# massquantity/LibRecommender

Hardware: NVIDIA H100
Metric: recommend_user users/sec (all-items top-K) (higher is better)
Workload: dtype f32 scores (fp16 tensor-core candidate pass + exact fp32 re-score)

## Files before the change

### librecommender_b200/csrc/score_topk_tc.cu

```cuda
#include <cmath>
#include <type_traits>
#include "common.cuh"
#include "ptx_sm90.cuh"
#include "../../include/b200reco.h"
#include <cuda_fp16.h>

namespace b200 {
namespace tc {

constexpr int TM = 128;
constexpr int TN = 256;
constexpr int KBLK = 64;
constexpr int CAPG_MAX = 256;
constexpr int GW = 8;
constexpr int REC = 12;
constexpr int NB = 1024;
constexpr int STEP = 64;
constexpr int W_PRE = 2;
constexpr int KROW_MAX = 288;
constexpr int MAX_KB = 4;
constexpr int PRE_STRIDE = 8;
constexpr double PRE_DELTA = 1e-5;
constexpr int PRE_TIE_ALLOWANCE = 16;
constexpr int A_KB_BYTES = TM * KBLK * 2;
constexpr int B_KB_BYTES = TN * KBLK * 2;
constexpr int MAXU = 3072;
constexpr int MAXC = 2048;
constexpr int FIN_THREADS = 256;
constexpr float ERR_COEF = 0.00097705f;

constexpr int SWEEP_CONSUMER_WARPS = 8;
constexpr int WARP_TMA = SWEEP_CONSUMER_WARPS;
constexpr int SWEEP_THREADS = 32 * (SWEEP_CONSUMER_WARPS + 4);
constexpr int SWEEP_PRODUCER_REGS = 40, SWEEP_CONSUMER_REGS = 232;

struct CatalogHeader {
  uint32_t max_norm_bits;
  int32_t d, d_pad;
  int64_t N, N_pad;
  float scale;
  float max_norm_scaled;
};

struct RowMeta {
  float eps2;
  float R;
  float scale;
  int32_t k_row;
  int32_t pre_k;
  int32_t active;
  int32_t apply;
  int32_t capped;
};


struct SweepParams {
  int64_t N;
  int32_t B_pad, m_tiles, n_splits, tiles_per_split, total_tiles, KB, nstage;
  int32_t kb_stages;
  int32_t n_pre_tiles;
  int32_t pre_stride;
  int32_t capg, trig;
  int32_t ablate;
  uint32_t hint_ns;
  const RowMeta* meta;
  uint32_t* row_tau_key;
  int32_t* row_status;
  uint32_t* ghist;
  float* cand_r;
  int32_t* cand_cnt;
  float* blockmax;
};

__device__ __forceinline__ float pow2_scale_for(float nrm) {
  if (!(nrm > 0.f) || !(nrm < 3.0e38f)) return 1.f;
  int x;
  frexpf(nrm, &x);
  int e = 7 - x;
  e = max(-120, min(120, e));
  return ldexpf(1.f, e);
}

__global__ void item_norm_kernel(const float* __restrict__ I, int64_t ldi, int64_t N, int d,
                                 CatalogHeader* hdr) {
  const int64_t row = ((int64_t)blockIdx.x * blockDim.x + threadIdx.x) >> 5;
  const int lane = threadIdx.x & 31;
  if (row >= N) return;
  float ss = 0.f;
  for (int k = lane; k < d; k += 32) {
    const float v = __ldg(I + row * ldi + k);
    ss = fmaf(v, v, ss);
  }
  ss = warp_sum(ss);
  if (lane == 0) atomicMax(&hdr->max_norm_bits, __float_as_uint(sqrtf(ss) * 1.0001f));
}

__global__ void item_scale_kernel(CatalogHeader* hdr) {
  const float mx = __uint_as_float(hdr->max_norm_bits);
  const float s = pow2_scale_for(mx);
  hdr->scale = s;
  hdr->max_norm_scaled = mx * s;
}

__global__ void prep_items_kernel(const float* __restrict__ I, int64_t ldi, int64_t N, int d,
                                  int d_pad, int64_t N_pad, __half* __restrict__ out,
                                  const CatalogHeader* __restrict__ hdr) {
  const int64_t row = ((int64_t)blockIdx.x * blockDim.x + threadIdx.x) >> 5;
  const int lane = threadIdx.x & 31;
  if (row >= N_pad) return;
  const float s = hdr->scale;
  for (int k = lane; k < d_pad; k += 32) {
// ... 534 lines not shown
      if (lane == 0) ptx::mbar_arrive(&ss->a_empty);
    }
  }
  __syncthreads();
  if (CL > 1) ptx::cluster_sync_all();
}

constexpr int GUESS_THREADS = 256;
__global__ void __launch_bounds__(GUESS_THREADS)
guess_kernel(const float* __restrict__ blockmax, int n_vals , int B_pad,
             const RowMeta* __restrict__ meta, uint32_t* __restrict__ row_tau_key,
             uint32_t* __restrict__ guess_key) {
  __shared__ uint32_t hist[32][256 + 1];
  __shared__ uint32_t s_prefix[32], s_krem[32], s_ok[32];
  const int lane = threadIdx.x & 31, wid = threadIdx.x >> 5;
  const int row = blockIdx.x * 32 + lane;
  const RowMeta m = meta[row];
  if (wid == 0) { s_prefix[lane] = 0; s_krem[lane] = (uint32_t)m.pre_k; s_ok[lane] = m.active != 0; }
  for (int pass = 0; pass < 4; ++pass) {
    const int shift = 24 - 8 * pass;
    for (int i = threadIdx.x; i < 32 * 257; i += GUESS_THREADS) (&hist[0][0])[i] = 0;
    __syncthreads();
    const uint32_t prefix = s_prefix[lane];
    for (int i = wid; i < n_vals; i += GUESS_THREADS / 32) {
      const float v = blockmax[(int64_t)i * B_pad + row];
      const uint32_t key = float_to_key(v);
      if (v > -3.0e38f && (pass == 0 || (key >> (shift + 8)) == prefix))
        atomicAdd(&hist[lane][(key >> shift) & 255u], 1u);
    }
    __syncthreads();
    for (int rr = wid; rr < 32; rr += GUESS_THREADS / 32) {
      uint32_t mine[8], tot = 0;
#pragma unroll
      for (int b = 0; b < 8; ++b) { mine[b] = hist[rr][lane * 8 + b]; tot += mine[b]; }
      uint32_t incl = tot;
#pragma unroll
      for (int o = 1; o < 32; o <<= 1) {
        const uint32_t t = __shfl_down_sync(0xffffffffu, incl, o);
        if (lane + o < 32) incl += t;
      }
      const uint32_t excl = incl - tot;
      const uint32_t krem = s_krem[rr];
      const uint32_t total = __shfl_sync(0xffffffffu, incl, 0);
      if (excl < krem && krem <= incl) {
        uint32_t c = excl;
#pragma unroll
        for (int b = 7; b >= 0; --b) {
          if (c + mine[b] >= krem) {
            s_prefix[rr] = (s_prefix[rr] << 8) | (uint32_t)(lane * 8 + b);
            s_krem[rr] = krem - c;
            break;
          }
          c += mine[b];
        }
      }
      if (lane == 0 && total < krem) s_ok[rr] = 0;
    }
    __syncthreads();
  }
  if (wid == 0) {
    const uint32_t key = s_ok[lane] ? s_prefix[lane] : 0u;
    row_tau_key[row] = key;
    guess_key[row] = key;
  }
}

struct FinalizeParams {
  int64_t B, N;
  int32_t B_pad, n_lists, K, d, capg;
  const RowMeta* meta;
  int32_t* row_status;
  const uint32_t* row_tau_key;
  const uint32_t* tau_guess_key;
  const float* cand_r;
  const int32_t* cand_cnt;
  const float* U; int64_t ldu;
  const float* I; int64_t ldi;
  const int64_t* user_ids;
  const int64_t* indptr; const int32_t* idx;
  int64_t* out_ids;
  float* out_scores;
};

__global__ void __launch_bounds__(FIN_THREADS, 5)
finalize_kernel(const FinalizeParams p) {
  __shared__ uint32_t hist[256];
  __shared__ uint32_t s_prefix, s_krem;
  __shared__ uint32_t s_wtot[FIN_THREADS / 32];
  __shared__ int s_nu, s_nc;
  __shared__ float u_s[MAXU];
  __shared__ int32_t u_id[MAXU];
  __shared__ unsigned long long c_sort[MAXC];
  __shared__ float urow[MAX_KB * KBLK];
  int32_t* htab = reinterpret_cast<int32_t*>(c_sort);
  const int tid = threadIdx.x;
  const int64_t row = blockIdx.x;
  int64_t* oid = p.out_ids + row * p.K;
  float* osc = p.out_scores ? p.out_scores + row * p.K : nullptr;
  const RowMeta meta = p.meta[row];
  auto give_up = [&](int code) {
    if (code && tid == 0) p.row_status[row] = code;
    for (int i = tid; i < p.K; i += FIN_THREADS) { oid[i] = -1; if (osc) osc[i] = 0.f; }
  };
  if (p.row_status[row] != 0) { give_up(0); return; }
  const uint32_t tk = p.row_tau_key[row];
  const float low = tk ? key_to_float(tk) : __int_as_float(0xff800000);
  if (tid == 0) { s_nu = 0; s_nc = 0; }
  int* s_cnt = reinterpret_cast<int*>(c_sort);
  int* s_off = s_cnt + p.n_lists;
  for (int s = tid; s < p.n_lists; s += FIN_THREADS) s_cnt[s] = p.cand_cnt[(int64_t)s * p.B_pad + row];
  __syncthreads();
  if (tid < 32) {
    const int per = (p.n_lists + 31) / 32;
    const int b = min(tid * per, p.n_lists), e = min(b + per, p.n_lists);
    int sum = 0;
    for (int s = b; s < e; ++s) sum += s_cnt[s];
    int incl = sum;
#pragma unroll
    for (int o = 1; o < 32; o <<= 1) {
      const int t = __shfl_up_sync(0xffffffffu, incl, o);
      if (tid >= o) incl += t;
    }
    int run = incl - sum;
    for (int s = b; s < e; ++s) { s_off[s] = run; run += s_cnt[s]; }
    if (tid == 31) s_off[p.n_lists] = incl;
  }
  __syncthreads();
  {
    const int lane = tid & 31;
    const int total = s_off[p.n_lists];
    constexpr int UN = 3;
    for (int g0 = 0; g0 < total; g0 += FIN_THREADS * UN) {
      float4 a[UN], b[UN];
      int base[UN];
      bool ok[UN];
#pragma unroll
      for (int q = 0; q < UN; ++q) {
        const int g = g0 + q * FIN_THREADS + tid;
        ok[q] = g < total;
        a[q] = b[q] = make_float4(0.f, 0.f, 0.f, 0.f);
        base[q] = 0;
        if (ok[q]) {
          int lo = 0, hi = p.n_lists - 1;
          while (lo < hi) {
            const int mid = (lo + hi + 1) >> 1;
            if (s_off[mid] <= g) lo = mid; else hi = mid - 1;
          }
          const int j = g - s_off[lo];
          const int64_t slot = (int64_t)lo * p.B_pad + row;
          const float4* ls = reinterpret_cast<const float4*>(p.cand_r + (slot * (int64_t)p.capg + j) * REC);
          a[q] = __ldcs(ls);
          b[q] = __ldcs(ls + 1);
          base[q] = __ldcs(reinterpret_cast<const int32_t*>(ls + 2));
        }
      }
#pragma unroll
      for (int q = 0; q < UN; ++q) {
        const float v[8] = {a[q].x, a[q].y, a[q].z, a[q].w, b[q].x, b[q].y, b[q].z, b[q].w};
#pragma unroll
        for (int e = 0; e < 8; ++e) {
          const bool hit = ok[q] && v[e] >= low && (int64_t)(base[q] + e) < p.N;
          const unsigned m = __ballot_sync(0xffffffffu, hit);
          if (m) {
            int pos0 = 0;
            if (lane == 0) pos0 = atomicAdd(&s_nu, __popc(m));
            pos0 = __shfl_sync(0xffffffffu, pos0, 0);
            const int pos = pos0 + __popc(m & ((1u << lane) - 1u));
            if (hit && pos < MAXU) { u_s[pos] = v[e]; u_id[pos] = base[q] + e; }
          }
        }
      }
    }
  }
  __syncthreads();
  const int nu = s_nu;
  if (nu < meta.k_row) { give_up(2); return; }
  const bool in_smem = nu <= MAXU;
  auto for_each = [&](auto&& f) {
    if (in_smem) {
      for (int i = tid; i < nu; i += FIN_THREADS) f(u_s[i], u_id[i]);
    } else {
      for (int s = 0; s < p.n_lists; ++s) {
        const int64_t slot = (int64_t)s * p.B_pad + row;
        const int n = p.cand_cnt[slot];
        const float* ls = p.cand_r + slot * (int64_t)(p.capg * REC);
        for (int i = tid; i < n * GW; i += FIN_THREADS) {
          const float v = ls[(i / GW) * REC + (i % GW)];
          const int32_t id = reinterpret_cast<const int32_t*>(ls)[(i / GW) * REC + 8] + (i % GW);
          if (v >= low && (int64_t)id < p.N) f(v, id);
        }
      }
    }
  };
  uint32_t prefix = 0, krem = (uint32_t)meta.k_row;
  for (int pass = 0; pass < 4; ++pass) {
    const int shift = 24 - 8 * pass;
    hist[tid] = 0;
    __syncthreads();
    for_each([&](float v, int32_t) {
      const uint32_t key = float_to_key(v);
      if (pass == 0 || (key >> (shift + 8)) == prefix) atomicAdd(&hist[(key >> shift) & 255u], 1u);
    });
    __syncthreads();
    {
      const int lane = tid & 31, wid = tid >> 5;
      const uint32_t v = hist[tid];
      uint32_t incl = v;
#pragma unroll
      for (int o = 1; o < 32; o <<= 1) {
        const uint32_t t = __shfl_down_sync(0xffffffffu, incl, o);
        if (lane + o < 32) incl += t;
      }
      if (lane == 0) s_wtot[wid] = incl;
      __syncthreads();
      uint32_t above = 0;
      for (int w2 = wid + 1; w2 < FIN_THREADS / 32; ++w2) above += s_wtot[w2];
      incl += above;
      const uint32_t excl = incl - v;
      if (excl < krem && krem <= incl) {
        s_prefix = (prefix << 8) | (uint32_t)tid;
        s_krem = krem - excl;
      }
    }
    __syncthreads();
    prefix = s_prefix;
    krem = s_krem;
    __syncthreads();
  }
  const float thr = key_to_float(prefix) - meta.eps2;
  {
    const uint32_t gk = p.tau_guess_key[row];
    if (gk != 0u && key_to_float(gk) > thr) { give_up(3); return; }
  }
  if (in_smem) {
    int my_keep[MAXU / FIN_THREADS];
#pragma unroll
    for (int t = 0; t < MAXU / FIN_THREADS; ++t) {
      const int i = tid + t * FIN_THREADS;
      my_keep[t] = (i < nu && u_s[i] >= thr) ? u_id[i] : -1;
    }
    __syncthreads();
#pragma unroll
    for (int t = 0; t < MAXU / FIN_THREADS; ++t) {
      if (my_keep[t] >= 0) {
        const int pos = atomicAdd(&s_nc, 1);
        if (pos < MAXC) u_id[pos] = my_keep[t];
      }
    }
  } else {
    __syncthreads();
    for_each([&](float v, int32_t id) {
      if (v >= thr) {
        const int pos = atomicAdd(&s_nc, 1);
        if (pos < MAXC) u_id[pos] = id;
      }
    });
  }
  for (int i = tid; i < 2 * MAXC; i += FIN_THREADS) htab[i] = -1;
  __syncthreads();
  const int nc = s_nc;
  int32_t* c_id = u_id;
  if (nc > MAXC || nc < p.K) { give_up(4); return; }
  const int64_t u = p.user_ids[row];
  if (meta.apply) {
    for (int i = tid; i < nc; i += FIN_THREADS) {
      uint32_t h = ((uint32_t)c_id[i] * 2654435761u) & (2 * MAXC - 1);
      while (atomicCAS(&htab[h], -1, i) != -1) h = (h + 1) & (2 * MAXC - 1);
    }
    __syncthreads();
    const int64_t beg = p.indptr[u], end = p.indptr[u + 1];
    for (int64_t j = beg + tid; j < end; j += FIN_THREADS) {
      const int32_t it = p.idx[j];
      uint32_t h = ((uint32_t)it * 2654435761u) & (2 * MAXC - 1);
      while (true) {
        const int32_t e = htab[h];
        if (e < 0) break;
        if (c_id[e] == it || c_id[e] == ~it) { c_id[e] = ~it; break; }
        h = (h + 1) & (2 * MAXC - 1);
      }
    }
  }
  for (int k = tid; k < p.d; k += FIN_THREADS) urow[k] = __ldg(p.U + u * p.ldu + k);
  __syncthreads();
  const bool vec4 = (p.d % 4 == 0) && (p.ldi % 4 == 0) && ((reinterpret_cast<uintptr_t>(p.I) & 15) == 0);
  int P = 1;
  while (P < nc) P <<= 1;
  unsigned long long mine[MAXC / FIN_THREADS];
#pragma unroll
  for (int t = 0; t < MAXC / FIN_THREADS; ++t) {
    const int i = tid + t * FIN_THREADS;
    unsigned long long comp = 0ull;
    if (i < nc && c_id[i] >= 0) {
      const float* it = p.I + (int64_t)c_id[i] * p.ldi;
      float acc = 0.f;
      if (vec4) {
        const float4* it4 = reinterpret_cast<const float4*>(it);
#pragma unroll 8
        for (int k4 = 0; k4 < p.d / 4; ++k4) {
          const float4 x = __ldg(it4 + k4);
          acc = fmaf(urow[4 * k4 + 0], x.x, acc);
          acc = fmaf(urow[4 * k4 + 1], x.y, acc);
          acc = fmaf(urow[4 * k4 + 2], x.z, acc);
          acc = fmaf(urow[4 * k4 + 3], x.w, acc);
        }
      } else {
        for (int k = 0; k < p.d; ++k) acc = fmaf(urow[k], __ldg(it + k), acc);
      }
      comp = ((unsigned long long)float_to_key(acc) << 32) | (unsigned long long)(~(uint32_t)c_id[i]);
    }
    mine[t] = comp;
  }
  __syncthreads();
  if (P <= 2 * FIN_THREADS) {
    auto bitonic_regs = [&](auto ec) {
      constexpr int EPT = decltype(ec)::value;
      unsigned long long x[EPT];
#pragma unroll
      for (int t = 0; t < EPT; ++t) x[t] = mine[t];
      int buf = 0;
#pragma unroll 1
      for (int k = 2; k <= P; k <<= 1) {
#pragma unroll 1
        for (int j = k >> 1; j > 0; j >>= 1) {
          if (EPT == 2 && j >= FIN_THREADS) {
            const unsigned long long a = x[0], b = x[EPT - 1];
            x[0] = a > b ? a : b;
            x[EPT - 1] = a > b ? b : a;
            continue;
          }
          unsigned long long y[EPT];
          if (j >= 32) {
            unsigned long long* sb = c_sort + buf * (EPT * FIN_THREADS);
#pragma unroll
            for (int t = 0; t < EPT; ++t) sb[t * FIN_THREADS + tid] = x[t];
            __syncthreads();
#pragma unroll
            for (int t = 0; t < EPT; ++t) y[t] = sb[t * FIN_THREADS + (tid ^ j)];
            buf ^= 1;
          } else {
#pragma unroll
            for (int t = 0; t < EPT; ++t) y[t] = __shfl_xor_sync(0xffffffffu, x[t], j);
          }
#pragma unroll
          for (int t = 0; t < EPT; ++t) {
            const int e = tid + t * FIN_THREADS;
            const bool take_max = (((e & k) == 0) == ((e & j) == 0));
            x[t] = take_max ? (x[t] > y[t] ? x[t] : y[t]) : (x[t] < y[t] ? x[t] : y[t]);
          }
        }
      }
      __syncthreads();
#pragma unroll
      for (int t = 0; t < EPT; ++t) c_sort[t * FIN_THREADS + tid] = x[t];
      __syncthreads();
    };
    if (P <= FIN_THREADS) bitonic_regs(std::integral_constant<int, 1>{});
    else bitonic_regs(std::integral_constant<int, 2>{});
  } else {
#pragma unroll
    for (int t = 0; t < MAXC / FIN_THREADS; ++t) {
      const int i = tid + t * FIN_THREADS;
      if (i < P) c_sort[i] = mine[t];
    }
    __syncthreads();
    for (int k = 2; k <= P; k <<= 1) {
      for (int j = k >> 1; j > 0; j >>= 1) {
        for (int i = tid; i < P; i += FIN_THREADS) {
          const int ixj = i ^ j;
          if (ixj > i) {
            const unsigned long long a = c_sort[i], b = c_sort[ixj];
            const bool desc = ((i & k) == 0);
            if (desc ? (a < b) : (a > b)) { c_sort[i] = b; c_sort[ixj] = a; }
          }
        }
        __syncthreads();
      }
    }
  }
  {
    const unsigned long long kth = c_sort[p.K - 1];
    const bool short_row = kth == 0ull;
    const bool unsafe = meta.capped && key_to_float((uint32_t)(kth >> 32)) * meta.scale < thr + 0.5f * meta.eps2;
    if (short_row || unsafe) { __syncthreads(); give_up(5); return; }
  }
  for (int i = tid; i < p.K; i += FIN_THREADS) {
    const unsigned long long c = c_sort[i];
    oid[i] = (int64_t)(~(uint32_t)(c & 0xffffffffull));
    if (osc) osc[i] = key_to_float((uint32_t)(c >> 32));
  }
}

typedef CUresult (*EncodeTiledFn)(CUtensorMap*, CUtensorMapDataType, cuuint32_t, void*,
                                  const cuuint64_t*, const cuuint64_t*, const cuuint32_t*,
                                  const cuuint32_t*, CUtensorMapInterleave, CUtensorMapSwizzle,
                                  CUtensorMapL2promotion, CUtensorMapFloatOOBfill);

static EncodeTiledFn get_encode_fn() {
  static EncodeTiledFn fn = nullptr;
  if (fn) return fn;
  void* p = nullptr;
  cudaDriverEntryPointQueryResult q;
  if (cudaGetDriverEntryPoint("cuTensorMapEncodeTiled", &p, cudaEnableDefault, &q) != cudaSuccess ||
      q != cudaDriverEntryPointSuccess)
    return nullptr;
  fn = (EncodeTiledFn)p;
  return fn;
}

static int make_tmap(CUtensorMap* m, const void* base, int64_t rows, int d_pad, int box_rows) {
  EncodeTiledFn enc = get_encode_fn();
  B200_REQUIRE(enc, "cuTensorMapEncodeTiled entry point not available");
  cuuint64_t dims[2] = {(cuuint64_t)d_pad, (cuuint64_t)rows};
  cuuint64_t strides[1] = {(cuuint64_t)d_pad * 2};
  cuuint32_t box[2] = {(cuuint32_t)KBLK, (cuuint32_t)box_rows};
  cuuint32_t estr[2] = {1, 1};
  CUresult r = enc(m, CU_TENSOR_MAP_DATA_TYPE_FLOAT16, 2, const_cast<void*>(base), dims, strides,
                   box, estr, CU_TENSOR_MAP_INTERLEAVE_NONE, CU_TENSOR_MAP_SWIZZLE_128B,
                   CU_TENSOR_MAP_L2_PROMOTION_L2_256B, CU_TENSOR_MAP_FLOAT_OOB_FILL_NONE);
  B200_REQUIRE(r == CUDA_SUCCESS, "cuTensorMapEncodeTiled failed (%d)", (int)r);
  return 0;
}

static inline int pad_to(int64_t x, int m) { return (int)((x + m - 1) / m * m); }
static inline size_t al256(size_t x) { return (x + 255) & ~(size_t)255; }


static int g_epi = 5;
static int g_cluster = 2;
static int g_nh = 1;
static int g_ablate = 0;
static int g_hint_ns = 20000;
static int g_pre_stride = PRE_STRIDE;
static double g_pre_delta = PRE_DELTA;
static float g_pre_coef = 0.f;
static int g_pre_margin = 12;

struct Plan {
  int B_pad, d_pad, KB, m_tiles, total_tiles, n_splits, tiles_per_split, nstage, n_pre_tiles, kb_stages;
  int W, n_lists, capg, trig;
  int CL, NH;
  bool use_pre;
  int pre_stride;
  int pre_sampled;
  int64_t N_pad;
  size_t smem_bytes;
  size_t off_A, off_meta, off_tau, off_guess, off_status, off_cnt, off_hist, off_cs, off_bm, total;
};

static int make_plan(int64_t B, int64_t N, int d, Plan* pl) {
  pl->d_pad = pad_to(d, KBLK);
  pl->KB = pl->d_pad / KBLK;
  B200_REQUIRE(pl->KB >= 1 && pl->KB <= MAX_KB, "fused scorer supports embed width <= %d (got %d)",
               MAX_KB * KBLK, d);
  pl->CL = (g_cluster == 2 && B > TM) ? 2 : 1;
  pl->kb_stages = pl->KB > 2;
  pl->NH = (g_nh == 3 && pl->kb_stages) ? 1 : g_nh;
  pl->B_pad = pad_to(B, TM * pl->CL);
  pl->N_pad = (N + TN - 1) / TN * TN;
  pl->m_tiles = pl->B_pad / TM;
  pl->total_tiles = (int)(pl->N_pad / TN);
  pl->W = 2;
  const int ovh = 12;
  long best = -1;
  int bestS = 1;
  const int sms = num_sms() > 0 ? num_sms() : 132;
  const int maxS = pl->total_tiles < 2 * sms ? pl->total_tiles : 2 * sms;
  for (int S = 1; S <= maxS; ++S) {
    const long units = (long)pl->m_tiles * S;
    const long waves = (units + sms - 1) / sms;
    const long tps = (pl->total_tiles + S - 1) / S;
    const long cost = waves * (tps + ovh);
// ... 199 lines not shown
  out[4] = pl.n_pre_tiles; out[5] = pl.nstage; out[6] = pl.CL * 10 + pl.NH; out[7] = pl.capg;
  if (n_out >= 10) { out[8] = pl.pre_stride; out[9] = pl.pre_sampled; }
  if (n_out >= 10 + KROW_MAX + 1) rank_table(pl, out + 10);
  return 0;
}

extern "C" int b200_recommend_embed_workspace_bytes(int64_t B, int64_t N, int32_t d, int32_t K,
                                                    size_t* bytes) {
  B200_REQUIRE(bytes && B >= 1 && N >= 1 && d >= 1 && K >= 1, "bad arguments");
  Plan pl;
  if (int rc = make_plan(B, N, d, &pl)) return rc;
  *bytes = pl.total;
  return 0;
}

extern "C" int b200_recommend_embed(const float* U, int64_t ldu, const int64_t* user_ids, int64_t B,
                                    const float* I, int64_t ldi, int64_t N, int32_t d,
                                    const void* catalog, const int64_t* indptr, const int32_t* idx,
                                    int64_t n_users, int32_t filter, int32_t K, int64_t* out_ids,
                                    float* out_scores, int32_t* row_status, void* workspace,
                                    size_t workspace_bytes, void* stream_, void* ev_sweep_start,
                                    void* ev_sweep_stop) {
  B200_REQUIRE(U && user_ids && I && catalog && out_ids && row_status && workspace,
               "b200_recommend_embed: null pointer");
  B200_REQUIRE((int64_t)K <= N, "`n_rec` %d exceeds num of items %lld", K, (long long)N);
  B200_REQUIRE(K <= KROW_MAX, "b200_recommend_embed: n_rec %d above the fused-path limit %d", K, KROW_MAX);
  B200_REQUIRE(N < (1ll << 31) - TN, "N too large");
  if (B == 0) return 0;
  cudaStream_t stream = (cudaStream_t)stream_;
  Plan pl;
  if (int rc = make_plan(B, N, d, &pl)) return rc;
  B200_REQUIRE(workspace_bytes >= pl.total, "workspace too small (%zu < %zu)", workspace_bytes, pl.total);
  char* ws = (char*)(((uintptr_t)workspace + 255) & ~(uintptr_t)255);
  __half* A = (__half*)(ws + pl.off_A);
  RowMeta* meta = (RowMeta*)(ws + pl.off_meta);
  uint32_t* tau = (uint32_t*)(ws + pl.off_tau);
  uint32_t* guess = (uint32_t*)(ws + pl.off_guess);
  int32_t* status = (int32_t*)(ws + pl.off_status);
  int32_t* cnt = (int32_t*)(ws + pl.off_cnt);
  uint32_t* ghist = (uint32_t*)(ws + pl.off_hist);
  float* cand_r = (float*)(ws + pl.off_cs);
  float* bm = (float*)(ws + pl.off_bm);
  const CatalogHeader* hdr = (const CatalogHeader*)catalog;
  const __half* Ih = (const __half*)((const char*)catalog + 256);

  PreRank pre_rank;
  rank_table(pl, pre_rank.k);
  prep_users_kernel<<<(unsigned)ceil_div64((int64_t)pl.B_pad * 32, 256), 256, 0, stream>>>(
      U, ldu, user_ids, B, pl.B_pad, d, pl.d_pad, K, N, filter, pre_rank, indptr, n_users, hdr, A, meta,
      tau, status);
  count_launch();
  B200_CUDA_OK(cudaMemsetAsync(cnt, 0, (pl.off_cs - pl.off_cnt), stream));

  CUtensorMap tmA, tmB, tmBh;
  if (int rc = make_tmap(&tmA, A, pl.B_pad, pl.d_pad, TM)) return rc;
  if (int rc = make_tmap(&tmB, Ih, pl.N_pad, pl.d_pad, TN)) return rc;
  if (int rc = make_tmap(&tmBh, Ih, pl.N_pad, pl.d_pad, TN / 2)) return rc;

  SweepParams sp;
  sp.N = N; sp.B_pad = pl.B_pad; sp.m_tiles = pl.m_tiles; sp.n_splits = pl.n_splits;
  sp.tiles_per_split = pl.tiles_per_split; sp.total_tiles = pl.total_tiles; sp.KB = pl.KB;
  sp.nstage = pl.nstage; sp.kb_stages = pl.kb_stages; sp.n_pre_tiles = pl.n_pre_tiles;
  sp.pre_stride = pl.pre_stride; sp.capg = pl.capg; sp.trig = pl.trig;
  sp.meta = meta; sp.row_tau_key = tau;
  sp.row_status = status; sp.ghist = ghist; sp.cand_r = cand_r; sp.cand_cnt = cnt;
  sp.blockmax = bm; sp.ablate = g_ablate; sp.hint_ns = (uint32_t)g_hint_ns;
  const int n_units = pl.m_tiles * pl.n_splits;
  const int sm_count = num_sms();
  int grid = n_units < sm_count ? n_units : sm_count;
  grid -= grid % pl.CL;

  if (ev_sweep_start) B200_CUDA_OK(cudaEventRecord((cudaEvent_t)ev_sweep_start, stream));
  if (pl.use_pre) {
    if (int rc = launch_pre_dispatch(grid, pl, stream, tmA, tmB, tmBh, sp)) return rc;
    guess_kernel<<<(unsigned)(pl.B_pad / 32), GUESS_THREADS, 0, stream>>>(
        bm, W_PRE * pl.n_splits * pl.n_pre_tiles, pl.B_pad, meta, tau, guess);
    count_launch();
  } else {
    B200_CUDA_OK(cudaMemsetAsync(guess, 0, (size_t)pl.B_pad * 4, stream));
  }
  if (int rc = launch_main_dispatch(grid, pl, g_epi, stream, tmA, tmB, tmBh, sp)) return rc;
  if (ev_sweep_stop) B200_CUDA_OK(cudaEventRecord((cudaEvent_t)ev_sweep_stop, stream));

  FinalizeParams fp;
  fp.B = B; fp.N = N; fp.B_pad = pl.B_pad; fp.n_lists = pl.n_lists; fp.K = K; fp.d = d; fp.capg = pl.capg;
  fp.meta = meta; fp.row_status = status; fp.row_tau_key = tau; fp.tau_guess_key = guess;
  fp.cand_r = cand_r; fp.cand_cnt = cnt;
  fp.U = U; fp.ldu = ldu; fp.I = I; fp.ldi = ldi; fp.user_ids = user_ids; fp.indptr = indptr;
  fp.idx = idx; fp.out_ids = out_ids; fp.out_scores = out_scores;
  finalize_kernel<<<(unsigned)B, FIN_THREADS, 0, stream>>>(fp);
  count_launch();
  B200_CUDA_OK(cudaMemcpyAsync(row_status, status, (size_t)B * 4, cudaMemcpyDeviceToDevice, stream));
  B200_CUDA_OK(cudaGetLastError());
  return 0;
}
```

Before: 2.343 million.

## Shrink finalize CTA, use min/max-bounded wide radix select, prefetch user row

The finalize kernel now runs 128-thread CTAs with 7 per SM and a smaller shared union buffer. The radix select starts from the common prefix of the observed min/max keys and uses 12-bit histograms stored in the sort buffer, so it needs fewer passes. The user embedding row and the first interaction id are loaded early to hide their latency, and the register bitonic sort is extended to 4 elements per thread. Rows with more than 1024 candidates now take the slower global-memory path, and the larger histograms add extra clearing and scanning work per pass.

```diff
diff --git a/librecommender_b200/csrc/score_topk_tc.cu b/librecommender_b200/csrc/score_topk_tc.cu
--- a/librecommender_b200/csrc/score_topk_tc.cu
+++ b/librecommender_b200/csrc/score_topk_tc.cu
@@ -24,9 +24,9 @@
 constexpr int PRE_TIE_ALLOWANCE = 16;
 constexpr int A_KB_BYTES = TM * KBLK * 2;
 constexpr int B_KB_BYTES = TN * KBLK * 2;
-constexpr int MAXU = 3072;
+constexpr int MAXU = 1024;
 constexpr int MAXC = 2048;
-constexpr int FIN_THREADS = 256;
+constexpr int FIN_THREADS = 128, FIN_CTAS_PER_SM = 7;
 constexpr float ERR_COEF = 0.00097705f;
 
 constexpr int SWEEP_CONSUMER_WARPS = 8;
@@ -727,30 +727,48 @@
   float* out_scores;
 };
 
-__global__ void __launch_bounds__(FIN_THREADS, 5)
+constexpr int SEL_BITS = 12;
+constexpr int SEL_BINS = 1 << SEL_BITS;
+static_assert(SEL_BINS * 4 <= MAXC * 8, "the select histogram lives in the sort buffer");
+static_assert(2 * MAXU >= MAXC, "the candidate ids live in the union buffer");
+static_assert(SEL_BINS % FIN_THREADS == 0, "whole bins per thread");
+constexpr int FIN_UR = (MAX_KB * KBLK + FIN_THREADS - 1) / FIN_THREADS;
+constexpr int FIN_SORT_REGS = 512;
+
+__global__ void __launch_bounds__(FIN_THREADS, FIN_CTAS_PER_SM)
 finalize_kernel(const FinalizeParams p) {
-  __shared__ uint32_t hist[256];
-  __shared__ uint32_t s_prefix, s_krem;
+  __shared__ uint32_t s_prefix, s_krem, s_kmin, s_kmax;
   __shared__ uint32_t s_wtot[FIN_THREADS / 32];
   __shared__ int s_nu, s_nc;
-  __shared__ float u_s[MAXU];
-  __shared__ int32_t u_id[MAXU];
-  __shared__ unsigned long long c_sort[MAXC];
+  __shared__ int32_t u_buf[2 * MAXU];
+  float* u_s = reinterpret_cast<float*>(u_buf);
+  int32_t* u_id = u_buf + MAXU;
+  __shared__ __align__(16) unsigned long long c_sort[MAXC];
   __shared__ float urow[MAX_KB * KBLK];
   int32_t* htab = reinterpret_cast<int32_t*>(c_sort);
+  uint32_t* hist = reinterpret_cast<uint32_t*>(c_sort);
   const int tid = threadIdx.x;
   const int64_t row = blockIdx.x;
   int64_t* oid = p.out_ids + row * p.K;
   float* osc = p.out_scores ? p.out_scores + row * p.K : nullptr;
+  const int64_t u = p.user_ids[row];
   const RowMeta meta = p.meta[row];
   auto give_up = [&](int code) {
     if (code && tid == 0) p.row_status[row] = code;
     for (int i = tid; i < p.K; i += FIN_THREADS) { oid[i] = -1; if (osc) osc[i] = 0.f; }
   };
   if (p.row_status[row] != 0) { give_up(0); return; }
+  float ur[FIN_UR];
+#pragma unroll
+  for (int t = 0; t < FIN_UR; ++t) {
+    const int k = tid + t * FIN_THREADS;
+    ur[t] = k < p.d ? __ldg(p.U + u * p.ldu + k) : 0.f;
+  }
+  int64_t cbeg = 0, cend = 0;
+  if (meta.apply) { cbeg = p.indptr[u]; cend = p.indptr[u + 1]; }
   const uint32_t tk = p.row_tau_key[row];
   const float low = tk ? key_to_float(tk) : __int_as_float(0xff800000);
-  if (tid == 0) { s_nu = 0; s_nc = 0; }
+  if (tid == 0) { s_nu = 0; s_nc = 0; s_kmin = 0xffffffffu; s_kmax = 0u; }
   int* s_cnt = reinterpret_cast<int*>(c_sort);
   int* s_off = s_cnt + p.n_lists;
   for (int s = tid; s < p.n_lists; s += FIN_THREADS) s_cnt[s] = p.cand_cnt[(int64_t)s * p.B_pad + row];
@@ -771,6 +789,7 @@
     if (tid == 31) s_off[p.n_lists] = incl;
   }
   __syncthreads();
+  uint32_t kmin = 0xffffffffu, kmax = 0u;
   {
     const int lane = tid & 31;
     const int total = s_off[p.n_lists];
@@ -805,6 +824,11 @@
 #pragma unroll
         for (int e = 0; e < 8; ++e) {
           const bool hit = ok[q] && v[e] >= low && (int64_t)(base[q] + e) < p.N;
+          if (hit) {
+            const uint32_t key = float_to_key(v[e]);
+            kmin = min(kmin, key);
+            kmax = max(kmax, key);
+          }
           const unsigned m = __ballot_sync(0xffffffffu, hit);
           if (m) {
             int pos0 = 0;
@@ -816,7 +840,15 @@
         }
       }
     }
-  }
+    kmin = __reduce_min_sync(0xffffffffu, kmin);
+    kmax = __reduce_max_sync(0xffffffffu, kmax);
+    if (lane == 0) { atomicMin(&s_kmin, kmin); atomicMax(&s_kmax, kmax); }
+  }
+#pragma unroll
+  for (int t = 0; t < FIN_UR; ++t)
+    if (tid + t * FIN_THREADS < p.d) urow[tid + t * FIN_THREADS] = ur[t];
+  const bool has_cid0 = cbeg + tid < cend;
+  const int32_t cid0 = has_cid0 ? p.idx[cbeg + tid] : 0;
   __syncthreads();
   const int nu = s_nu;
   if (nu < meta.k_row) { give_up(2); return; }
@@ -837,19 +869,27 @@
       }
     }
   };
-  uint32_t prefix = 0, krem = (uint32_t)meta.k_row;
-  for (int pass = 0; pass < 4; ++pass) {
-    const int shift = 24 - 8 * pass;
-    hist[tid] = 0;
+  uint32_t krem = (uint32_t)meta.k_row;
+  int rem = 32 - __clz(s_kmin ^ s_kmax);
+  uint32_t prefix = rem == 32 ? 0u : s_kmax >> rem;
+  while (rem > 0) {
+    const int w = min(SEL_BITS, rem), shift = rem - w;
+    for (int i = tid; i < SEL_BINS; i += FIN_THREADS) hist[i] = 0;
     __syncthreads();
     for_each([&](float v, int32_t) {
       const uint32_t key = float_to_key(v);
-      if (pass == 0 || (key >> (shift + 8)) == prefix) atomicAdd(&hist[(key >> shift) & 255u], 1u);
+      if (rem == 32 || (key >> rem) == prefix) atomicAdd(&hist[(key >> shift) & ((1u << w) - 1u)], 1u);
     });
     __syncthreads();
     {
+      constexpr int BPT = SEL_BINS / FIN_THREADS;
       const int lane = tid & 31, wid = tid >> 5;
-      const uint32_t v = hist[tid];
+      uint32_t v = 0;
+#pragma unroll
+      for (int b = 0; b < BPT; b += 4) {
+        const uint4 q = *reinterpret_cast<const uint4*>(hist + tid * BPT + b);
+        v += q.x + q.y + q.z + q.w;
+      }
       uint32_t incl = v;
 #pragma unroll
       for (int o = 1; o < 32; o <<= 1) {
@@ -861,61 +901,60 @@
       uint32_t above = 0;
       for (int w2 = wid + 1; w2 < FIN_THREADS / 32; ++w2) above += s_wtot[w2];
       incl += above;
-      const uint32_t excl = incl - v;
+      uint32_t excl = incl - v;
       if (excl < krem && krem <= incl) {
-        s_prefix = (prefix << 8) | (uint32_t)tid;
-        s_krem = krem - excl;
+#pragma unroll
+        for (int b = BPT - 1; b >= 0; --b) {
+          const uint32_t c = hist[tid * BPT + b];
+          if (excl + c >= krem) {
+            s_prefix = (prefix << w) | (uint32_t)(tid * BPT + b);
+            s_krem = krem - excl;
+            break;
+          }
+          excl += c;
+        }
       }
     }
     __syncthreads();
     prefix = s_prefix;
     krem = s_krem;
-    __syncthreads();
+    rem = shift;
   }
   const float thr = key_to_float(prefix) - meta.eps2;
   {
     const uint32_t gk = p.tau_guess_key[row];
     if (gk != 0u && key_to_float(gk) > thr) { give_up(3); return; }
   }
+  int32_t* c_id = u_buf;
   if (in_smem) {
-    int my_keep[MAXU / FIN_THREADS];
-#pragma unroll
-    for (int t = 0; t < MAXU / FIN_THREADS; ++t) {
-      const int i = tid + t * FIN_THREADS;
-      my_keep[t] = (i < nu && u_s[i] >= thr) ? u_id[i] : -1;
-    }
-    __syncthreads();
-#pragma unroll
-    for (int t = 0; t < MAXU / FIN_THREADS; ++t) {
-      if (my_keep[t] >= 0) {
+    for (int i0 = 0; i0 < nu; i0 += FIN_THREADS) {
+      const int i = i0 + tid;
+      const int32_t keep = (i < nu && u_s[i] >= thr) ? u_id[i] : -1;
+      __syncthreads();
+      if (keep >= 0) {
         const int pos = atomicAdd(&s_nc, 1);
-        if (pos < MAXC) u_id[pos] = my_keep[t];
+        if (pos < MAXC) c_id[pos] = keep;
       }
     }
   } else {
-    __syncthreads();
     for_each([&](float v, int32_t id) {
       if (v >= thr) {
         const int pos = atomicAdd(&s_nc, 1);
-        if (pos < MAXC) u_id[pos] = id;
+        if (pos < MAXC) c_id[pos] = id;
       }
     });
   }
   for (int i = tid; i < 2 * MAXC; i += FIN_THREADS) htab[i] = -1;
   __syncthreads();
   const int nc = s_nc;
-  int32_t* c_id = u_id;
   if (nc > MAXC || nc < p.K) { give_up(4); return; }
-  const int64_t u = p.user_ids[row];
   if (meta.apply) {
     for (int i = tid; i < nc; i += FIN_THREADS) {
       uint32_t h = ((uint32_t)c_id[i] * 2654435761u) & (2 * MAXC - 1);
       while (atomicCAS(&htab[h], -1, i) != -1) h = (h + 1) & (2 * MAXC - 1);
     }
     __syncthreads();
-    const int64_t beg = p.indptr[u], end = p.indptr[u + 1];
-    for (int64_t j = beg + tid; j < end; j += FIN_THREADS) {
-      const int32_t it = p.idx[j];
+    auto remove = [&](int32_t it) {
       uint32_t h = ((uint32_t)it * 2654435761u) & (2 * MAXC - 1);
       while (true) {
         const int32_t e = htab[h];
@@ -923,17 +962,15 @@
         if (c_id[e] == it || c_id[e] == ~it) { c_id[e] = ~it; break; }
         h = (h + 1) & (2 * MAXC - 1);
       }
-    }
-  }
-  for (int k = tid; k < p.d; k += FIN_THREADS) urow[k] = __ldg(p.U + u * p.ldu + k);
+    };
+    if (has_cid0) remove(cid0);
+    for (int64_t j = cbeg + FIN_THREADS + tid; j < cend; j += FIN_THREADS) remove(p.idx[j]);
+  }
   __syncthreads();
   const bool vec4 = (p.d % 4 == 0) && (p.ldi % 4 == 0) && ((reinterpret_cast<uintptr_t>(p.I) & 15) == 0);
   int P = 1;
   while (P < nc) P <<= 1;
-  unsigned long long mine[MAXC / FIN_THREADS];
-#pragma unroll
-  for (int t = 0; t < MAXC / FIN_THREADS; ++t) {
-    const int i = tid + t * FIN_THREADS;
+  for (int i = tid; i < P; i += FIN_THREADS) {
     unsigned long long comp = 0ull;
     if (i < nc && c_id[i] >= 0) {
       const float* it = p.I + (int64_t)c_id[i] * p.ldi;
@@ -953,24 +990,33 @@
       }
       comp = ((unsigned long long)float_to_key(acc) << 32) | (unsigned long long)(~(uint32_t)c_id[i]);
     }
-    mine[t] = comp;
+    c_sort[i] = comp;
   }
   __syncthreads();
-  if (P <= 2 * FIN_THREADS) {
+  if (P <= FIN_SORT_REGS) {
     auto bitonic_regs = [&](auto ec) {
       constexpr int EPT = decltype(ec)::value;
       unsigned long long x[EPT];
 #pragma unroll
-      for (int t = 0; t < EPT; ++t) x[t] = mine[t];
+      for (int t = 0; t < EPT; ++t) x[t] = tid + t * FIN_THREADS < P ? c_sort[tid + t * FIN_THREADS] : 0ull;
       int buf = 0;
 #pragma unroll 1
       for (int k = 2; k <= P; k <<= 1) {
 #pragma unroll 1
         for (int j = k >> 1; j > 0; j >>= 1) {
-          if (EPT == 2 && j >= FIN_THREADS) {
-            const unsigned long long a = x[0], b = x[EPT - 1];
-            x[0] = a > b ? a : b;
-            x[EPT - 1] = a > b ? b : a;
+          if (EPT > 1 && j >= FIN_THREADS) {
+#pragma unroll
+            for (int t = 0; t < EPT; ++t) {
+#pragma unroll
+              for (int t2 = t + 1; t2 < EPT; ++t2) {
+                if ((t ^ t2) * FIN_THREADS == j) {
+                  const unsigned long long a = x[t], b = x[t2];
+                  const bool desc = ((tid + t * FIN_THREADS) & k) == 0;
+                  x[t] = desc == (a > b) ? a : b;
+                  x[t2] = desc == (a > b) ? b : a;
+                }
+              }
+            }
             continue;
           }
           unsigned long long y[EPT];
@@ -1000,14 +1046,9 @@
       __syncthreads();
     };
     if (P <= FIN_THREADS) bitonic_regs(std::integral_constant<int, 1>{});
-    else bitonic_regs(std::integral_constant<int, 2>{});
+    else if (P <= 2 * FIN_THREADS) bitonic_regs(std::integral_constant<int, 2>{});
+    else if constexpr (4 * FIN_THREADS <= FIN_SORT_REGS) bitonic_regs(std::integral_constant<int, 4>{});
   } else {
-#pragma unroll
-    for (int t = 0; t < MAXC / FIN_THREADS; ++t) {
-      const int i = tid + t * FIN_THREADS;
-      if (i < P) c_sort[i] = mine[t];
-    }
-    __syncthreads();
     for (int k = 2; k <= P; k <<= 1) {
       for (int j = k >> 1; j > 0; j >>= 1) {
         for (int i = tid; i < P; i += FIN_THREADS) {
```

After: 2.372 million (median of 6 runs). About the same (+1.2%).

## Rework finalize kernel: smaller smem footprint, adaptive radix select, async prefetches

Applied to the files above, without the earlier changes.

Shrinks the finalize kernel's shared memory by overlaying candidate ids, scores, sort keys and hash table in one pool, and raises launch bounds from 5 to 6 blocks per SM. The radix select now tracks the min and max key of the surviving candidates and only histograms the bits that actually differ, which can mean fewer passes than the fixed four. The user embedding row, indptr bounds and the user's seen-item list are prefetched with cp.async so their loads overlap the candidate gather. Rescoring is computed lazily instead of through a per-thread array, and the fixed register array in compaction is replaced by a chunked loop. The cost is an added cap on the number of lists per row and a more complex shared-memory aliasing scheme.

```diff
diff --git a/librecommender_b200/csrc/score_topk_tc.cu b/librecommender_b200/csrc/score_topk_tc.cu
--- a/librecommender_b200/csrc/score_topk_tc.cu
+++ b/librecommender_b200/csrc/score_topk_tc.cu
@@ -727,39 +727,68 @@
   float* out_scores;
 };
 
-__global__ void __launch_bounds__(FIN_THREADS, 5)
+__device__ __forceinline__ void cp_async4(void* dst, const void* src) {
+  asm volatile("cp.async.ca.shared.global [%0], [%1], 4;"
+               ::"r"((uint32_t)__cvta_generic_to_shared(dst)), "l"(src) : "memory");
+}
+__device__ __forceinline__ void cp_async8(void* dst, const void* src) {
+  asm volatile("cp.async.ca.shared.global [%0], [%1], 8;"
+               ::"r"((uint32_t)__cvta_generic_to_shared(dst)), "l"(src) : "memory");
+}
+__device__ __forceinline__ void cp_async_wait_all() { asm volatile("cp.async.wait_all;" ::: "memory"); }
+
+constexpr int FIN_IDX_STAGE = 256;
+constexpr int FIN_MAX_LISTS = 767;
+
+__global__ void __launch_bounds__(FIN_THREADS, 6)
 finalize_kernel(const FinalizeParams p) {
-  __shared__ uint32_t hist[256];
-  __shared__ uint32_t s_prefix, s_krem;
+  __shared__ __align__(16) uint32_t s_scr[256 + FIN_MAX_LISTS + 1];
+  uint32_t* hist = s_scr;
+  int32_t* s_idx = reinterpret_cast<int32_t*>(s_scr + 256);
+  int* s_off = reinterpret_cast<int*>(s_scr + 256);
+  __shared__ uint32_t s_prefix, s_krem, s_kmin, s_kmax;
   __shared__ uint32_t s_wtot[FIN_THREADS / 32];
   __shared__ int s_nu, s_nc;
-  __shared__ float u_s[MAXU];
-  __shared__ int32_t u_id[MAXU];
-  __shared__ unsigned long long c_sort[MAXC];
+  __shared__ int64_t s_u, s_beg, s_end;
+  __shared__ uint32_t s_gk;
+  __shared__ RowMeta s_meta;
+  __shared__ __align__(16) int32_t s_pool[2 * MAXU];
+  static_assert(2 * MAXU - MAXC >= 2 * MAXC, "hash set / sort keys must fit behind the candidate ids");
+  int32_t* u_id = s_pool;
+  float* u_s = reinterpret_cast<float*>(s_pool + MAXU);
+  unsigned long long* c_sort = reinterpret_cast<unsigned long long*>(s_pool + MAXC);
   __shared__ float urow[MAX_KB * KBLK];
   int32_t* htab = reinterpret_cast<int32_t*>(c_sort);
   const int tid = threadIdx.x;
   const int64_t row = blockIdx.x;
-  int64_t* oid = p.out_ids + row * p.K;
-  float* osc = p.out_scores ? p.out_scores + row * p.K : nullptr;
-  const RowMeta meta = p.meta[row];
   auto give_up = [&](int code) {
+    cp_async_wait_all();
     if (code && tid == 0) p.row_status[row] = code;
-    for (int i = tid; i < p.K; i += FIN_THREADS) { oid[i] = -1; if (osc) osc[i] = 0.f; }
+    for (int i = tid; i < p.K; i += FIN_THREADS) {
+      p.out_ids[row * p.K + i] = -1;
+      if (p.out_scores) p.out_scores[row * p.K + i] = 0.f;
+    }
   };
-  if (p.row_status[row] != 0) { give_up(0); return; }
+  const int status = p.row_status[row];
   const uint32_t tk = p.row_tau_key[row];
+  const RowMeta& meta = s_meta;
+  if (tid == 0) {
+    s_nu = 0; s_nc = 0; s_kmin = 0xffffffffu; s_kmax = 0u;
+    s_u = p.user_ids[row]; s_gk = p.tau_guess_key[row]; s_meta = p.meta[row];
+  }
+  hist[tid] = 0;
+  for (int s = tid; s < p.n_lists; s += FIN_THREADS) s_off[s] = p.cand_cnt[(int64_t)s * p.B_pad + row];
+  __syncthreads();
+  if (status != 0) { give_up(0); return; }
+  const int64_t u = s_u;
+  if (tid < p.d) cp_async4(&urow[tid], p.U + u * p.ldu + tid);
+  if (meta.apply && tid == 32) { cp_async8(&s_beg, p.indptr + u); cp_async8(&s_end, p.indptr + u + 1); }
   const float low = tk ? key_to_float(tk) : __int_as_float(0xff800000);
-  if (tid == 0) { s_nu = 0; s_nc = 0; }
-  int* s_cnt = reinterpret_cast<int*>(c_sort);
-  int* s_off = s_cnt + p.n_lists;
-  for (int s = tid; s < p.n_lists; s += FIN_THREADS) s_cnt[s] = p.cand_cnt[(int64_t)s * p.B_pad + row];
-  __syncthreads();
   if (tid < 32) {
     const int per = (p.n_lists + 31) / 32;
     const int b = min(tid * per, p.n_lists), e = min(b + per, p.n_lists);
     int sum = 0;
-    for (int s = b; s < e; ++s) sum += s_cnt[s];
+    for (int s = b; s < e; ++s) sum += s_off[s];
     int incl = sum;
 #pragma unroll
     for (int o = 1; o < 32; o <<= 1) {
@@ -767,14 +796,15 @@
       if (tid >= o) incl += t;
     }
     int run = incl - sum;
-    for (int s = b; s < e; ++s) { s_off[s] = run; run += s_cnt[s]; }
+    for (int s = b; s < e; ++s) { const int c = s_off[s]; s_off[s] = run; run += c; }
     if (tid == 31) s_off[p.n_lists] = incl;
   }
   __syncthreads();
   {
     const int lane = tid & 31;
     const int total = s_off[p.n_lists];
-    constexpr int UN = 3;
+    uint32_t kmin = 0xffffffffu, kmax = 0u;
+    constexpr int UN = 2;
     for (int g0 = 0; g0 < total; g0 += FIN_THREADS * UN) {
       float4 a[UN], b[UN];
       int base[UN];
@@ -811,15 +841,26 @@
             if (lane == 0) pos0 = atomicAdd(&s_nu, __popc(m));
             pos0 = __shfl_sync(0xffffffffu, pos0, 0);
             const int pos = pos0 + __popc(m & ((1u << lane) - 1u));
-            if (hit && pos < MAXU) { u_s[pos] = v[e]; u_id[pos] = base[q] + e; }
+            if (hit) {
+              const uint32_t key = float_to_key(v[e]);
+              kmin = min(kmin, key);
+              kmax = max(kmax, key);
+              if (pos < MAXU) { u_s[pos] = v[e]; u_id[pos] = base[q] + e; }
+            }
           }
         }
       }
     }
-  }
+    kmin = __reduce_min_sync(0xffffffffu, kmin);
+    kmax = __reduce_max_sync(0xffffffffu, kmax);
+    if (lane == 0) { atomicMin(&s_kmin, kmin); atomicMax(&s_kmax, kmax); }
+  }
+  cp_async_wait_all();
   __syncthreads();
   const int nu = s_nu;
   if (nu < meta.k_row) { give_up(2); return; }
+  if (meta.apply && s_end - s_beg <= FIN_IDX_STAGE)
+    for (int j = tid; j < (int)(s_end - s_beg); j += FIN_THREADS) cp_async4(&s_idx[j], p.idx + s_beg + j);
   const bool in_smem = nu <= MAXU;
   auto for_each = [&](auto&& f) {
     if (in_smem) {
@@ -837,19 +878,22 @@
       }
     }
   };
+  const uint32_t kmin = s_kmin;
+  const uint32_t span = s_kmax - kmin;
+  const int bits = span ? 32 - __clz(span) : 0;
   uint32_t prefix = 0, krem = (uint32_t)meta.k_row;
-  for (int pass = 0; pass < 4; ++pass) {
-    const int shift = 24 - 8 * pass;
-    hist[tid] = 0;
-    __syncthreads();
+  for (int hb = bits; hb > 0;) {
+    const int w = min(8, hb), shift = hb - w;
+    const bool first = hb == bits;
     for_each([&](float v, int32_t) {
-      const uint32_t key = float_to_key(v);
-      if (pass == 0 || (key >> (shift + 8)) == prefix) atomicAdd(&hist[(key >> shift) & 255u], 1u);
+      const uint32_t o = float_to_key(v) - kmin;
+      if (first || (o >> hb) == prefix) atomicAdd(&hist[(o >> shift) & ((1u << w) - 1u)], 1u);
     });
     __syncthreads();
     {
       const int lane = tid & 31, wid = tid >> 5;
       const uint32_t v = hist[tid];
+      hist[tid] = 0;
       uint32_t incl = v;
 #pragma unroll
       for (int o = 1; o < 32; o <<= 1) {
@@ -863,33 +907,33 @@
       incl += above;
       const uint32_t excl = incl - v;
       if (excl < krem && krem <= incl) {
-        s_prefix = (prefix << 8) | (uint32_t)tid;
+        s_prefix = (prefix << w) | (uint32_t)tid;
         s_krem = krem - excl;
       }
     }
     __syncthreads();
     prefix = s_prefix;
     krem = s_krem;
-    __syncthreads();
-  }
-  const float thr = key_to_float(prefix) - meta.eps2;
-  {
-    const uint32_t gk = p.tau_guess_key[row];
-    if (gk != 0u && key_to_float(gk) > thr) { give_up(3); return; }
-  }
+    hb = shift;
+  }
+  const float thr = key_to_float(kmin + prefix) - meta.eps2;
+  if (s_gk != 0u && key_to_float(s_gk) > thr) { give_up(3); return; }
   if (in_smem) {
-    int my_keep[MAXU / FIN_THREADS];
-#pragma unroll
-    for (int t = 0; t < MAXU / FIN_THREADS; ++t) {
-      const int i = tid + t * FIN_THREADS;
-      my_keep[t] = (i < nu && u_s[i] >= thr) ? u_id[i] : -1;
-    }
-    __syncthreads();
-#pragma unroll
-    for (int t = 0; t < MAXU / FIN_THREADS; ++t) {
-      if (my_keep[t] >= 0) {
-        const int pos = atomicAdd(&s_nc, 1);
-        if (pos < MAXC) u_id[pos] = my_keep[t];
+    constexpr int CH = 4;
+    for (int r0 = 0; r0 < nu; r0 += CH * FIN_THREADS) {
+      int keep[CH];
+#pragma unroll
+      for (int t = 0; t < CH; ++t) {
+        const int i = r0 + t * FIN_THREADS + tid;
+        keep[t] = (i < nu && u_s[i] >= thr) ? u_id[i] : -1;
+      }
+      __syncthreads();
+#pragma unroll
+      for (int t = 0; t < CH; ++t) {
+        if (keep[t] >= 0) {
+          const int pos = atomicAdd(&s_nc, 1);
+          if (pos < MAXC) u_id[pos] = keep[t];
+        }
       }
     }
   } else {
@@ -902,20 +946,21 @@
     });
   }
   for (int i = tid; i < 2 * MAXC; i += FIN_THREADS) htab[i] = -1;
+  cp_async_wait_all();
   __syncthreads();
   const int nc = s_nc;
   int32_t* c_id = u_id;
   if (nc > MAXC || nc < p.K) { give_up(4); return; }
-  const int64_t u = p.user_ids[row];
   if (meta.apply) {
     for (int i = tid; i < nc; i += FIN_THREADS) {
       uint32_t h = ((uint32_t)c_id[i] * 2654435761u) & (2 * MAXC - 1);
       while (atomicCAS(&htab[h], -1, i) != -1) h = (h + 1) & (2 * MAXC - 1);
     }
     __syncthreads();
-    const int64_t beg = p.indptr[u], end = p.indptr[u + 1];
+    const int64_t beg = s_beg, end = s_end;
+    const bool staged = end - beg <= FIN_IDX_STAGE;
     for (int64_t j = beg + tid; j < end; j += FIN_THREADS) {
-      const int32_t it = p.idx[j];
+      const int32_t it = staged ? s_idx[j - beg] : p.idx[j];
       uint32_t h = ((uint32_t)it * 2654435761u) & (2 * MAXC - 1);
       while (true) {
         const int32_t e = htab[h];
@@ -925,43 +970,35 @@
       }
     }
   }
-  for (int k = tid; k < p.d; k += FIN_THREADS) urow[k] = __ldg(p.U + u * p.ldu + k);
   __syncthreads();
   const bool vec4 = (p.d % 4 == 0) && (p.ldi % 4 == 0) && ((reinterpret_cast<uintptr_t>(p.I) & 15) == 0);
   int P = 1;
   while (P < nc) P <<= 1;
-  unsigned long long mine[MAXC / FIN_THREADS];
-#pragma unroll
-  for (int t = 0; t < MAXC / FIN_THREADS; ++t) {
-    const int i = tid + t * FIN_THREADS;
-    unsigned long long comp = 0ull;
-    if (i < nc && c_id[i] >= 0) {
-      const float* it = p.I + (int64_t)c_id[i] * p.ldi;
-      float acc = 0.f;
-      if (vec4) {
-        const float4* it4 = reinterpret_cast<const float4*>(it);
+  auto score = [&](int i) -> unsigned long long {
+    if (i >= nc || c_id[i] < 0) return 0ull;
+    const float* it = p.I + (int64_t)c_id[i] * p.ldi;
+    float acc = 0.f;
+    if (vec4) {
+      const float4* it4 = reinterpret_cast<const float4*>(it);
 #pragma unroll 8
-        for (int k4 = 0; k4 < p.d / 4; ++k4) {
-          const float4 x = __ldg(it4 + k4);
-          acc = fmaf(urow[4 * k4 + 0], x.x, acc);
-          acc = fmaf(urow[4 * k4 + 1], x.y, acc);
-          acc = fmaf(urow[4 * k4 + 2], x.z, acc);
-          acc = fmaf(urow[4 * k4 + 3], x.w, acc);
-        }
-      } else {
-        for (int k = 0; k < p.d; ++k) acc = fmaf(urow[k], __ldg(it + k), acc);
-      }
-      comp = ((unsigned long long)float_to_key(acc) << 32) | (unsigned long long)(~(uint32_t)c_id[i]);
-    }
-    mine[t] = comp;
-  }
-  __syncthreads();
+      for (int k4 = 0; k4 < p.d / 4; ++k4) {
+        const float4 x = __ldg(it4 + k4);
+        acc = fmaf(urow[4 * k4 + 0], x.x, acc);
+        acc = fmaf(urow[4 * k4 + 1], x.y, acc);
+        acc = fmaf(urow[4 * k4 + 2], x.z, acc);
+        acc = fmaf(urow[4 * k4 + 3], x.w, acc);
+      }
+    } else {
+      for (int k = 0; k < p.d; ++k) acc = fmaf(urow[k], __ldg(it + k), acc);
+    }
+    return ((unsigned long long)float_to_key(acc) << 32) | (unsigned long long)(~(uint32_t)c_id[i]);
+  };
   if (P <= 2 * FIN_THREADS) {
     auto bitonic_regs = [&](auto ec) {
       constexpr int EPT = decltype(ec)::value;
       unsigned long long x[EPT];
 #pragma unroll
-      for (int t = 0; t < EPT; ++t) x[t] = mine[t];
+      for (int t = 0; t < EPT; ++t) x[t] = score(tid + t * FIN_THREADS);
       int buf = 0;
 #pragma unroll 1
       for (int k = 2; k <= P; k <<= 1) {
@@ -1002,11 +1039,7 @@
     if (P <= FIN_THREADS) bitonic_regs(std::integral_constant<int, 1>{});
     else bitonic_regs(std::integral_constant<int, 2>{});
   } else {
-#pragma unroll
-    for (int t = 0; t < MAXC / FIN_THREADS; ++t) {
-      const int i = tid + t * FIN_THREADS;
-      if (i < P) c_sort[i] = mine[t];
-    }
+    for (int i = tid; i < P; i += FIN_THREADS) c_sort[i] = score(i);
     __syncthreads();
     for (int k = 2; k <= P; k <<= 1) {
       for (int j = k >> 1; j > 0; j >>= 1) {
@@ -1030,8 +1063,8 @@
   }
   for (int i = tid; i < p.K; i += FIN_THREADS) {
     const unsigned long long c = c_sort[i];
-    oid[i] = (int64_t)(~(uint32_t)(c & 0xffffffffull));
-    if (osc) osc[i] = key_to_float((uint32_t)(c >> 32));
+    p.out_ids[row * p.K + i] = (int64_t)(~(uint32_t)(c & 0xffffffffull));
+    if (p.out_scores) p.out_scores[row * p.K + i] = key_to_float((uint32_t)(c >> 32));
   }
 }
 
@@ -1397,6 +1430,8 @@
   if (int rc = launch_main_dispatch(grid, pl, g_epi, stream, tmA, tmB, tmBh, sp)) return rc;
   if (ev_sweep_stop) B200_CUDA_OK(cudaEventRecord((cudaEvent_t)ev_sweep_stop, stream));
 
+  B200_REQUIRE(pl.n_lists <= FIN_MAX_LISTS, "b200_recommend_embed: %d candidate lists per row exceed %d",
+               pl.n_lists, FIN_MAX_LISTS);
   FinalizeParams fp;
   fp.B = B; fp.N = N; fp.B_pad = pl.B_pad; fp.n_lists = pl.n_lists; fp.K = K; fp.d = d; fp.capg = pl.capg;
   fp.meta = meta; fp.row_status = status; fp.row_tau_key = tau; fp.tau_guess_key = guess;
```

Result: faster. 2.357 million before, 2.452 million after (median of 6 runs) (+4.0%).
